# facebookresearch/flashy

Hardware: AMD Instinct MI355X
Metric: img/sec (higher is better)
Workload: dtype bf16; 1 GPU; model=resnet18, dataset=cifar10-shaped, global_batch=64, img_size=32, num_classes=10, parallelism=dp1, mode=native-kernels, graph=True, channels_last=False

## Files before the change

### flashy_amd/nn.py

```python
from __future__ import annotations

import math
import os
import typing as tp

import torch
from torch import nn

from . import ops


def _weight_bf16(w: torch.Tensor) -> torch.Tensor:
    mirror = getattr(w, "_bf16_mirror", None)
    if mirror is not None:
        return mirror
    return w.detach().to(torch.bfloat16)


def _grad_target(p: torch.Tensor) -> tp.Tuple[torch.Tensor, bool]:
    if p.grad is not None and p.grad.is_contiguous():
        return p.grad, True
    return torch.zeros_like(p, memory_format=torch.contiguous_format), False


# ... 63 lines not shown
                             self._wt_view, self.feeds_bn and self.training)


class WtCache:

    def __init__(self, model: nn.Module):
        convs = [m for m in model.modules()
                 if isinstance(m, Conv2d) and m.input_grad
                 and m.weight.shape[-1] % 64 == 0]
        metas, total = [], 0
        mirrors = [getattr(c.weight, "_bf16_mirror", None) for c in convs]
        if not convs or any(m is None for m in mirrors):
            self.meta = None
            return
        base = mirrors[0]
        for c, mir in zip(convs, mirrors):
            assert mir.untyped_storage().data_ptr() == \
                base.untyped_storage().data_ptr(), \
                "all conv weights must share one flat bf16 mirror"
            src_off = (mir.data_ptr() - base.data_ptr()) // 2
            assert src_off >= 0
            K, R, S, C = c.weight.shape
            metas.append((src_off, total, K, R * S * C))
            total += K * R * S * C
        dev = convs[0].weight.device
        self.src = mirrors[0]
        self.arena = torch.empty(total, dtype=torch.bfloat16, device=dev)
        self.meta = torch.tensor([list(m) for m in metas],
                                 dtype=torch.int32, device=dev).flatten()
        self.max_elems = max(m[2] * m[3] for m in metas)
        self.n = len(convs)
        for c, m in zip(convs, metas):
            K, R, S, C = c.weight.shape
            c._wt_view = self.arena[m[1]:m[1] + K * R * S * C].view(R, S, C, K)

    @property
    def active(self) -> bool:
        return self.meta is not None

    def refresh(self) -> None:
        if self.meta is not None:
            ops.weight_transpose_batched(self.src, self.arena, self.meta,
                                         self.n, self.max_elems)


class _BnFn(torch.autograd.Function):
    @staticmethod
    def forward(ctx, x: torch.Tensor, gamma: torch.Tensor, beta: torch.Tensor,
                res: tp.Optional[torch.Tensor], relu: bool, slope: float,
                module):
        N, H, W, C = x.shape
        M = N * H * W
        y = torch.empty_like(x)
        if module.training:
            fused = getattr(x, "_bn_stats", None)
            if fused is not None:
                partials, msplit = fused
            else:
                msplit = ops.bn_msplit(M, C)
                partials = torch.empty(msplit * 2 * C, dtype=torch.float32,
                                       device=x.device)
                ops.bn_stats(x, partials, M, C, msplit)
            work = torch.empty(4 * C, dtype=torch.float32, device=x.device)
            ops.bn_finalize(partials, msplit, gamma, beta, module.running_mean,
                            module.running_var, work, M, C, module.eps,
                            module.momentum, update_running=True)
        else:
            invstd = torch.rsqrt(module.running_var + module.eps)
            scale = gamma.detach() * invstd
            shift = beta.detach() - module.running_mean * scale
            work = torch.cat([module.running_mean, invstd, scale, shift])
        ops.bn_apply(x, res, y, work, M, C, relu, slope)
        ctx.save_for_backward(x, y, work)
        ctx.relu = relu
        ctx.slope = slope
        ctx.has_res = res is not None
        ctx.refs = (gamma, beta)
        return y

    @staticmethod
    def backward(ctx, dy: torch.Tensor):
        x, y, work = ctx.saved_tensors
        gamma, beta = ctx.refs
        N, H, W, C = x.shape
        M = N * H * W
        dy = dy.contiguous()
        msplit = ops.bn_msplit(M, C)
        partials = torch.empty(msplit * 2 * C, dtype=torch.float32,
                               device=x.device)
        bsums = torch.empty(2 * C, dtype=torch.float32, device=x.device)
        dz = torch.empty_like(dy)
        ops.bn_bwd_reduce(dy, y, x, work, dz, partials, M, C, msplit,
                          ctx.relu, ctx.slope)
        need_g, need_b = ctx.needs_input_grad[1], ctx.needs_input_grad[2]
        dgamma, g_direct = _grad_target(gamma) if need_g \
            else (torch.empty_like(gamma), True)
        dbeta, b_direct = _grad_target(beta) if need_b \
            else (torch.empty_like(beta), True)
        ops.bn_bwd_grads(partials, msplit, bsums, dgamma, dbeta, C)
        dx = torch.empty_like(x)
        ops.bn_bwd_apply(dz, x, work, bsums, dx, M, C)
        return (dx,
                dgamma if need_g and not g_direct else None,
                dbeta if need_b and not b_direct else None,
                dz if ctx.has_res else None,
                None, None, None)


class _ConvTransposeFn(torch.autograd.Function):

    @staticmethod
    def forward(ctx, x: torch.Tensor, w: torch.Tensor, stride: int, pad: int,
                input_grad: bool):
        w16 = _weight_bf16(w)
        N, Hi, Wi, Cin = x.shape
        K, R, S, Cout = w16.shape
        assert K == Cin, (x.shape, w16.shape)
        Ho = (Hi - 1) * stride - 2 * pad + R
        Wo = (Wi - 1) * stride - 2 * pad + S
        d = ops.ConvDims(N, Ho, Wo, Cout, Cin, R, S, Hi, Wi, stride, pad)
        y = x.new_empty((N, Ho, Wo, Cout))
        if Cout % 64 == 0:
            wt = w16.new_empty((R, S, Cout, Cin))
            ops.weight_transpose(w16, wt)
            ops.conv_dgrad(x, wt, y, d)
        else:
            ops.conv_stem_dgrad(x, w16, y, d)
        ctx.save_for_backward(x, w16)
        ctx.dims = d
        ctx.input_grad = input_grad
        ctx.w_ref = w
        return y

    @staticmethod
    def backward(ctx, dy: torch.Tensor):
        x, w16 = ctx.saved_tensors
        d: ops.ConvDims = ctx.dims
        dy = dy.contiguous()
        dw_buf = None
        direct = True
        if ctx.needs_input_grad[1]:
            dw_buf, direct = _grad_target(ctx.w_ref)
            ops.conv_wgrad(dy, x, dw_buf, d)
        dx = None
        if ctx.input_grad:
            dx = x.new_empty(x.shape)
            ops.conv_fwd(dy, w16, dx, d)
        return (dx, dw_buf if dw_buf is not None and not direct else None,
                None, None, None)


class ConvTranspose2d(nn.Module):

    def __init__(self, in_channels: int, out_channels: int, kernel_size: int,
# ... 220 lines not shown
```

### flashy_amd/ops/__init__.py

```python
from __future__ import annotations

import importlib.util
import math
import os
import typing as tp
from pathlib import Path

import torch

_ext = None
_load_error: tp.Optional[str] = None


def _find_so() -> tp.Optional[Path]:
    for pattern in ("_hip_ops*.so",):
        hits = sorted(Path(__file__).parent.glob(pattern))
        if hits:
            return hits[0]
    return None


def load_extension():
    global _ext, _load_error
    if _ext is not None:
# ... 631 lines not shown
        ext.conv_stem_wgrad(x.data_ptr(), dout.data_ptr(), dw.data_ptr(), *d,
                            _stream())



def bn_msplit(M: int, C: int) -> int:
    cols = max(1, C // 64)
    msplit = max(1, min(512 // cols, 512))
    msplit = max(1, min(msplit, (M + 31) // 32))
    if msplit >= 4:
        msplit &= ~3
    return msplit


def bn_stats(x: torch.Tensor, partials: torch.Tensor, M: int, C: int,
             msplit: int) -> None:
    require().bn_stats(x.data_ptr(), partials.data_ptr(), M, C, msplit, _stream())


def bn_finalize(partials, msplit: int, gamma, beta, rmean, rvar, work,
                M: int, C: int, eps: float, momentum: float,
                update_running: bool) -> None:
    require().bn_finalize(partials.data_ptr(), msplit, gamma.data_ptr(),
                          beta.data_ptr(), rmean.data_ptr(), rvar.data_ptr(),
                          work.data_ptr(), M, C, eps, momentum,
                          update_running, _stream())


def bn_apply(x, res, y, work, M: int, C: int, relu: bool,
             slope: float = 0.0) -> None:
    require().bn_apply(x.data_ptr(), res.data_ptr() if res is not None else 0,
                       y.data_ptr(), work.data_ptr(), M, C, relu, slope,
                       _stream())


def bn_bwd_reduce(dy, y, x, work, dz_out, partials, M: int, C: int,
                  msplit: int, relu: bool, slope: float = 0.0) -> None:
    require().bn_bwd_reduce(dy.data_ptr(), y.data_ptr(), x.data_ptr(),
                            work.data_ptr(), dz_out.data_ptr(),
                            partials.data_ptr(), M, C, msplit, relu, slope,
                            _stream())


def bn_bwd_grads(partials, msplit: int, bsums, dgamma, dbeta, C: int) -> None:
    require().bn_bwd_grads(partials.data_ptr(), msplit, bsums.data_ptr(),
                           dgamma.data_ptr(), dbeta.data_ptr(), C, _stream())


def bn_bwd_apply(dz, x, work, bsums, dx, M: int, C: int) -> None:
    require().bn_bwd_apply(dz.data_ptr(), x.data_ptr(), work.data_ptr(),
                           bsums.data_ptr(), dx.data_ptr(), M, C, _stream())



def cross_entropy_fwd_bwd(logits: torch.Tensor, target: torch.Tensor,
                          dlogits: torch.Tensor, loss_sum: torch.Tensor,
                          loss_scale: float, grad_scale: float) -> None:
    ext = require()
    B, C = logits.shape
    assert logits.is_contiguous() and target.dtype == torch.int64
    ext.cross_entropy(logits.data_ptr(), target.data_ptr(), dlogits.data_ptr(),
                      loss_sum.data_ptr(), B, C, loss_scale, grad_scale,
                      _is_bf16(logits), _stream())


def cross_entropy_mix_fwd_bwd(logits: torch.Tensor, target: torch.Tensor,
                              target_b: tp.Optional[torch.Tensor],
                              lam: tp.Optional[torch.Tensor],
                              dlogits: torch.Tensor, loss_sum: torch.Tensor,
                              label_smoothing: float, loss_scale: float,
                              grad_scale: float) -> None:
    ext = require()
    B, C = logits.shape
    assert logits.is_contiguous() and logits.is_cuda
    assert dlogits.is_contiguous() and dlogits.dtype == logits.dtype
    assert tuple(dlogits.shape) == (B, C)
    for t in (target, target_b):
        if t is not None:
            assert t.dtype == torch.int64 and tuple(t.shape) == (B,)
            assert t.is_contiguous() and t.device == logits.device
    if lam is not None:
        assert lam.dtype == torch.float32 and lam.numel() == 1
        assert lam.device == logits.device
    assert 0.0 <= label_smoothing <= 1.0, label_smoothing
    ext.cross_entropy_mix(logits.data_ptr(), target.data_ptr(),
                          target_b.data_ptr() if target_b is not None else 0,
                          lam.data_ptr() if lam is not None else 0,
                          dlogits.data_ptr(), loss_sum.data_ptr(), B, C,
                          float(label_smoothing), loss_scale, grad_scale,
                          _is_bf16(logits), _stream())


def bce_logits_fwd_bwd(x: torch.Tensor, dx: torch.Tensor,
                       loss_sum: torch.Tensor, target: float,
                       loss_scale: float, grad_scale: float) -> None:
    ext = require()
    assert x.is_contiguous()
    ext.bce_logits(x.data_ptr(), dx.data_ptr(), loss_sum.data_ptr(), x.numel(),
                   target, loss_scale, grad_scale, _is_bf16(x), _stream())


def mse_fwd_bwd(x: torch.Tensor, t: torch.Tensor, dx: torch.Tensor,
                loss_sum: torch.Tensor, loss_scale: float,
                grad_scale: float) -> None:
    ext = require()
    assert x.is_contiguous() and t.is_contiguous() and x.dtype == t.dtype
# ... 88 lines not shown
```

### flashy_amd/ops/csrc/batchnorm.hip

```cpp

#include "common.h"


__global__ void __launch_bounds__(256)
k_bn_stats(const uint16_t* __restrict__ x, float* __restrict__ partials,
           int64_t M, int C, int msplit, int m_per_block) {
    const int c8 = (threadIdx.x & 7) * 8;
    const int mlane = threadIdx.x >> 3;
    const int cbase = blockIdx.x * 64;
    const int64_t m0 = (int64_t)blockIdx.y * m_per_block;
    const int64_t m1 = min(m0 + (int64_t)m_per_block, M);
    float s[8] = {}, s2[8] = {};
    for (int64_t m = m0 + mlane; m < m1; m += 32) {
        const short8 v8 = *reinterpret_cast<const short8*>(
            x + m * C + cbase + c8);
#pragma unroll
        for (int j = 0; j < 8; ++j) {
            const float v = bf16_to_f32(((const uint16_t*)&v8)[j]);
            s[j] += v;
            s2[j] = fmaf(v, v, s2[j]);
        }
    }
    __shared__ float red[2][32][64];
#pragma unroll
// ... 2 lines not shown
        red[1][mlane][c8 + j] = s2[j];
    }
    __syncthreads();
    const int c = threadIdx.x & 63;
    const int which = threadIdx.x >> 6;
    if (which < 2) {
        float acc = 0.f;
#pragma unroll 8
        for (int i = 0; i < 32; ++i) acc += red[which][i][c];
        partials[((int64_t)which * C + cbase + c) * msplit + blockIdx.y] = acc;
    }
}


__device__ __forceinline__ void combine_partials8(
        const float* __restrict__ partials, int msplit, int C,
        float* s_out, float* s2_out) {
    const int ch = threadIdx.x & 7;
    const int slane = threadIdx.x >> 3;
    const int c = blockIdx.x * 8 + ch;
    const float* row0 = partials + (int64_t)c * msplit;
    const float* row1 = partials + ((int64_t)C + c) * msplit;
    float s = 0.f, s2 = 0.f;
    if (msplit & 3) {
        for (int i = slane; i < msplit; i += 32) {
            s += row0[i];
            s2 += row1[i];
        }
    } else {
        for (int i = slane * 4; i + 4 <= msplit; i += 128) {
            const float4 a = *reinterpret_cast<const float4*>(row0 + i);
            const float4 b = *reinterpret_cast<const float4*>(row1 + i);
            s += a.x + a.y + a.z + a.w;
            s2 += b.x + b.y + b.z + b.w;
        }
    }
    __shared__ float red[2][32][8];
    red[0][slane][ch] = s;
    red[1][slane][ch] = s2;
    __syncthreads();
    if (threadIdx.x < 16) {
        const int w = threadIdx.x >> 3;
        const int cc = threadIdx.x & 7;
        float acc = 0.f;
#pragma unroll 8
        for (int i = 0; i < 32; ++i) acc += red[w][i][cc];
        red[w][0][cc] = acc;
    }
    __syncthreads();
    *s_out = red[0][0][ch];
    *s2_out = red[1][0][ch];
}

__global__ void __launch_bounds__(256)
k_bn_finalize(const float* __restrict__ partials, int msplit,
              const float* __restrict__ gamma,
              const float* __restrict__ beta,
              float* __restrict__ running_mean,
              float* __restrict__ running_var,
              float* __restrict__ work, int64_t M, int C,
              float eps, float momentum, int update_running) {
    float s, s2;
    combine_partials8(partials, msplit, C, &s, &s2);
    if (threadIdx.x >= 8) return;
    const int c = blockIdx.x * 8 + threadIdx.x;
    const float mean = s / (float)M;
    float var = s2 / (float)M - mean * mean;
    var = fmaxf(var, 0.f);
    const float invstd = rsqrtf(var + eps);
    const float scale = gamma[c] * invstd;
    work[c] = mean;
    work[C + c] = invstd;
    work[2 * C + c] = scale;
    work[3 * C + c] = beta[c] - mean * scale;
    if (update_running) {
        running_mean[c] += momentum * (mean - running_mean[c]);
        const float unbiased = M > 1 ? var * (float)M / (float)(M - 1) : var;
        running_var[c] += momentum * (unbiased - running_var[c]);
    }
}


template <bool RELU, bool RES>
__global__ void __launch_bounds__(256)
k_bn_apply(const uint16_t* __restrict__ x, const uint16_t* __restrict__ res,
           uint16_t* __restrict__ y, const float* __restrict__ work,
           int64_t M, int C, float slope) {
    const int64_t total8 = M * C / 8;
    const int64_t stride = (int64_t)gridDim.x * blockDim.x;
    const float4* scale4 = reinterpret_cast<const float4*>(work + 2 * (int64_t)C);
    const float4* shift4 = reinterpret_cast<const float4*>(work + 3 * (int64_t)C);
    for (int64_t i = (int64_t)blockIdx.x * blockDim.x + threadIdx.x; i < total8;
         i += stride) {
        const int co = (int)((i * 8) % C) / 4;
        const float4 sc[2] = {scale4[co], scale4[co + 1]};
        const float4 sh[2] = {shift4[co], shift4[co + 1]};
        short8 xv = *reinterpret_cast<const short8*>(x + i * 8);
        short8 rv = {};
        if (RES) rv = *reinterpret_cast<const short8*>(res + i * 8);
        short8 out;
#pragma unroll
        for (int j = 0; j < 8; ++j) {
            float v = fmaf(bf16_to_f32(((const uint16_t*)&xv)[j]),
                           ((const float*)sc)[j], ((const float*)sh)[j]);
            if (RES) v += bf16_to_f32(((const uint16_t*)&rv)[j]);
            if (RELU) v = v > 0.f ? v : slope * v;
            ((uint16_t*)&out)[j] = f32_to_bf16(v);
        }
        *reinterpret_cast<short8*>(y + i * 8) = out;
    }
}

template <bool RELU, bool RES>
__global__ void __launch_bounds__(256)
k_bn_apply_c64(const uint16_t* __restrict__ x, const uint16_t* __restrict__ res,
               uint16_t* __restrict__ y, const float* __restrict__ work,
               int64_t M, int C, float slope, int m_per_block) {
    const int c = blockIdx.x * 64 + (threadIdx.x & 7) * 8;
    const int mlane = threadIdx.x >> 3;
    const int64_t m0 = (int64_t)blockIdx.y * m_per_block;
    const int64_t m1 = min(m0 + (int64_t)m_per_block, M);
    float sc[8], sh[8];
#pragma unroll
    for (int j = 0; j < 8; ++j) {
        sc[j] = work[2 * (int64_t)C + c + j];
        sh[j] = work[3 * (int64_t)C + c + j];
    }
    for (int64_t m = m0 + mlane; m < m1; m += 32) {
        const int64_t off = m * C + c;
        short8 xv = *reinterpret_cast<const short8*>(x + off);
        short8 rv = {};
        if (RES) rv = *reinterpret_cast<const short8*>(res + off);
        short8 out;
#pragma unroll
        for (int j = 0; j < 8; ++j) {
            float v = fmaf(bf16_to_f32(((const uint16_t*)&xv)[j]), sc[j], sh[j]);
            if (RES) v += bf16_to_f32(((const uint16_t*)&rv)[j]);
            if (RELU) v = v > 0.f ? v : slope * v;
            ((uint16_t*)&out)[j] = f32_to_bf16(v);
        }
        *reinterpret_cast<short8*>(y + off) = out;
    }
}

__global__ void __launch_bounds__(256)
k_bn_bwd_apply_c64(const uint16_t* __restrict__ dz,
                   const uint16_t* __restrict__ x,
                   const float* __restrict__ work,
                   const float* __restrict__ bsums,
                   uint16_t* __restrict__ dx, int64_t M, int C,
                   int m_per_block) {
    const int c = blockIdx.x * 64 + (threadIdx.x & 7) * 8;
    const int mlane = threadIdx.x >> 3;
    const int64_t m0 = (int64_t)blockIdx.y * m_per_block;
    const int64_t m1 = min(m0 + (int64_t)m_per_block, M);
    const float invM = 1.f / (float)M;
    float mn[8], is[8], sc[8], b0[8], b1[8];
#pragma unroll
    for (int j = 0; j < 8; ++j) {
        mn[j] = work[c + j];
        is[j] = work[C + c + j];
        sc[j] = work[2 * (int64_t)C + c + j];
        b0[j] = bsums[c + j] * invM;
        b1[j] = bsums[C + c + j] * invM;
    }
    for (int64_t m = m0 + mlane; m < m1; m += 32) {
        const int64_t off = m * C + c;
        short8 gz = *reinterpret_cast<const short8*>(dz + off);
        short8 xv = *reinterpret_cast<const short8*>(x + off);
        short8 out;
#pragma unroll
        for (int j = 0; j < 8; ++j) {
            const float xhat = (bf16_to_f32(((const uint16_t*)&xv)[j]) - mn[j])
                               * is[j];
            const float g = bf16_to_f32(((const uint16_t*)&gz)[j]);
            ((uint16_t*)&out)[j] =
                f32_to_bf16(sc[j] * (g - b0[j] - xhat * b1[j]));
        }
        *reinterpret_cast<short8*>(dx + off) = out;
    }
}

static inline int apply_mpb(int64_t M, int C) {
    const int cblocks = C / 64;
    int target = 1024 / cblocks;
    if (target < 1) target = 1;
    int64_t mblocks = (M + 31) / 32;
    if (mblocks > target) mblocks = target;
    return (int)((M + mblocks - 1) / mblocks);
}


template <bool RELU>
__global__ void __launch_bounds__(256)
k_bn_bwd_reduce(const uint16_t* __restrict__ dy, const uint16_t* __restrict__ y,
                const uint16_t* __restrict__ x, const float* __restrict__ work,
                uint16_t* __restrict__ dz_out, float* __restrict__ partials,
                int64_t M, int C, int msplit, int m_per_block, float slope) {
    const int c8 = (threadIdx.x & 7) * 8;
    const int mlane = threadIdx.x >> 3;
    const int cbase = blockIdx.x * 64;
    const int64_t m0 = (int64_t)blockIdx.y * m_per_block;
    const int64_t m1 = min(m0 + (int64_t)m_per_block, M);
    float mean[8], invstd[8];
#pragma unroll
    for (int j = 0; j < 8; ++j) {
        mean[j] = work[cbase + c8 + j];
        invstd[j] = work[C + cbase + c8 + j];
    }
    float s[8] = {}, sx[8] = {};
    for (int64_t m = m0 + mlane; m < m1; m += 32) {
        const int64_t off = m * C + cbase + c8;
        const short8 g8 = *reinterpret_cast<const short8*>(dy + off);
        const short8 x8 = *reinterpret_cast<const short8*>(x + off);
        short8 y8 = {};
        if (RELU) y8 = *reinterpret_cast<const short8*>(y + off);
        short8 dz8;
#pragma unroll
        for (int j = 0; j < 8; ++j) {
            float g = bf16_to_f32(((const uint16_t*)&g8)[j]);
            if (RELU && bf16_to_f32(((const uint16_t*)&y8)[j]) <= 0.f)
                g *= slope;
            ((uint16_t*)&dz8)[j] = f32_to_bf16(g);
            s[j] += g;
            const float xh = (bf16_to_f32(((const uint16_t*)&x8)[j]) - mean[j]) * invstd[j];
            sx[j] = fmaf(g, xh, sx[j]);
        }
        *reinterpret_cast<short8*>(dz_out + off) = dz8;
    }
    __shared__ float red[2][32][64];
#pragma unroll
// ... 11 lines not shown
        partials[((int64_t)which * C + cbase + c) * msplit + blockIdx.y] = acc;
    }
}

__global__ void __launch_bounds__(256)
k_bn_bwd_grads(const float* __restrict__ partials, int msplit,
               float* __restrict__ bsums,
               float* __restrict__ dgamma,
               float* __restrict__ dbeta, int C) {
    float s, sx;
    combine_partials8(partials, msplit, C, &s, &sx);
    if (threadIdx.x >= 8) return;
    const int c = blockIdx.x * 8 + threadIdx.x;
    bsums[c] = s;
    bsums[C + c] = sx;
    dbeta[c] += s;
    dgamma[c] += sx;
}


__global__ void __launch_bounds__(256)
k_bn_bwd_apply(const uint16_t* __restrict__ dz, const uint16_t* __restrict__ x,
               const float* __restrict__ work, const float* __restrict__ bsums,
               uint16_t* __restrict__ dx, int64_t M, int C) {
    const int64_t total8 = M * C / 8;
    const int64_t stride = (int64_t)gridDim.x * blockDim.x;
    const float invM = 1.f / (float)M;
    const float4* mean4 = reinterpret_cast<const float4*>(work);
    const float4* invstd4 = reinterpret_cast<const float4*>(work + C);
    const float4* scale4 = reinterpret_cast<const float4*>(work + 2 * (int64_t)C);
    const float4* b04 = reinterpret_cast<const float4*>(bsums);
    const float4* b14 = reinterpret_cast<const float4*>(bsums + C);
    for (int64_t i = (int64_t)blockIdx.x * blockDim.x + threadIdx.x; i < total8;
         i += stride) {
        const int co = (int)((i * 8) % C) / 4;
        const float4 mn[2] = {mean4[co], mean4[co + 1]};
        const float4 is[2] = {invstd4[co], invstd4[co + 1]};
        const float4 sc[2] = {scale4[co], scale4[co + 1]};
        const float4 b0[2] = {b04[co], b04[co + 1]};
        const float4 b1[2] = {b14[co], b14[co + 1]};
        short8 gz = *reinterpret_cast<const short8*>(dz + i * 8);
        short8 xv = *reinterpret_cast<const short8*>(x + i * 8);
        short8 out;
#pragma unroll
        for (int j = 0; j < 8; ++j) {
            const float xhat = (bf16_to_f32(((const uint16_t*)&xv)[j]) -
                                ((const float*)mn)[j]) * ((const float*)is)[j];
            const float g = bf16_to_f32(((const uint16_t*)&gz)[j]);
            const float v = ((const float*)sc)[j] *
                (g - (((const float*)b0)[j] + xhat * ((const float*)b1)[j]) * invM);
            ((uint16_t*)&out)[j] = f32_to_bf16(v);
        }
        *reinterpret_cast<short8*>(dx + i * 8) = out;
    }
}


extern "C" void launch_bn_stats(const void* x, void* partials, int64_t M, int C,
                                int msplit, hipStream_t stream) {
    const int mpb = (int)((M + msplit - 1) / msplit);
    dim3 grid((unsigned)(C / 64), (unsigned)msplit);
    k_bn_stats<<<grid, 256, 0, stream>>>((const uint16_t*)x, (float*)partials,
                                         M, C, msplit, mpb);
}

extern "C" void launch_bn_finalize(const void* partials, int msplit,
                                   const void* gamma, const void* beta,
                                   void* running_mean, void* running_var,
                                   void* work, int64_t M, int C, float eps,
                                   float momentum, int update_running,
                                   hipStream_t stream) {
    k_bn_finalize<<<C / 8, 256, 0, stream>>>(
        (const float*)partials, msplit, (const float*)gamma,
        (const float*)beta, (float*)running_mean, (float*)running_var,
        (float*)work, M, C, eps, momentum, update_running);
}

extern "C" void launch_bn_apply(const void* x, const void* res, void* y,
                                const void* work, int64_t M, int C, int relu,
                                float slope, hipStream_t stream) {
    if (C % 64 == 0) {
        const int mpb = apply_mpb(M, C);
        dim3 g((unsigned)(C / 64), (unsigned)((M + mpb - 1) / mpb));
        if (relu && res)
            k_bn_apply_c64<true, true><<<g, 256, 0, stream>>>(
                (const uint16_t*)x, (const uint16_t*)res, (uint16_t*)y,
                (const float*)work, M, C, slope, mpb);
        else if (relu)
            k_bn_apply_c64<true, false><<<g, 256, 0, stream>>>(
                (const uint16_t*)x, nullptr, (uint16_t*)y,
                (const float*)work, M, C, slope, mpb);
        else if (res)
            k_bn_apply_c64<false, true><<<g, 256, 0, stream>>>(
                (const uint16_t*)x, (const uint16_t*)res, (uint16_t*)y,
                (const float*)work, M, C, slope, mpb);
        else
            k_bn_apply_c64<false, false><<<g, 256, 0, stream>>>(
                (const uint16_t*)x, nullptr, (uint16_t*)y,
                (const float*)work, M, C, slope, mpb);
        return;
    }
    const int grid = ew_grid(M * C / 8, 256, 4);
    if (relu && res)
        k_bn_apply<true, true><<<grid, 256, 0, stream>>>(
            (const uint16_t*)x, (const uint16_t*)res, (uint16_t*)y,
            (const float*)work, M, C, slope);
// ... 3 lines not shown
    else if (res)
        k_bn_apply<false, true><<<grid, 256, 0, stream>>>(
            (const uint16_t*)x, (const uint16_t*)res, (uint16_t*)y,
            (const float*)work, M, C, slope);
    else
        k_bn_apply<false, false><<<grid, 256, 0, stream>>>(
            (const uint16_t*)x, nullptr, (uint16_t*)y, (const float*)work, M, C, slope);
}

extern "C" void launch_bn_bwd_reduce(const void* dy, const void* y,
                                     const void* x, const void* work,
                                     void* dz_out, void* partials, int64_t M,
                                     int C, int msplit, int relu, float slope,
                                     hipStream_t stream) {
    const int mpb = (int)((M + msplit - 1) / msplit);
    dim3 grid((unsigned)(C / 64), (unsigned)msplit);
    if (relu)
        k_bn_bwd_reduce<true><<<grid, 256, 0, stream>>>(
            (const uint16_t*)dy, (const uint16_t*)y, (const uint16_t*)x,
            (const float*)work, (uint16_t*)dz_out, (float*)partials, M, C,
            msplit, mpb, slope);
    else
        k_bn_bwd_reduce<false><<<grid, 256, 0, stream>>>(
            (const uint16_t*)dy, (const uint16_t*)y, (const uint16_t*)x,
            (const float*)work, (uint16_t*)dz_out, (float*)partials, M, C,
            msplit, mpb, slope);
}

extern "C" void launch_bn_bwd_grads(const void* partials, int msplit,
                                    void* bsums, void* dgamma, void* dbeta,
                                    int C, hipStream_t stream) {
    k_bn_bwd_grads<<<C / 8, 256, 0, stream>>>(
        (const float*)partials, msplit, (float*)bsums, (float*)dgamma,
        (float*)dbeta, C);
}

extern "C" void launch_bn_bwd_apply(const void* dz, const void* x,
                                    const void* work, const void* bsums,
                                    void* dx, int64_t M, int C,
                                    hipStream_t stream) {
    if (C % 64 == 0) {
        const int mpb = apply_mpb(M, C);
        dim3 g((unsigned)(C / 64), (unsigned)((M + mpb - 1) / mpb));
        k_bn_bwd_apply_c64<<<g, 256, 0, stream>>>(
            (const uint16_t*)dz, (const uint16_t*)x, (const float*)work,
            (const float*)bsums, (uint16_t*)dx, M, C, mpb);
        return;
    }
    const int grid = ew_grid(M * C / 8, 256, 4);
    k_bn_bwd_apply<<<grid, 256, 0, stream>>>(
        (const uint16_t*)dz, (const uint16_t*)x, (const float*)work,
        (const float*)bsums, (uint16_t*)dx, M, C);
}
```

### flashy_amd/ops/csrc/ext.cpp

```cpp

#include <hip/hip_runtime.h>
#include <pybind11/pybind11.h>
#include <pybind11/stl.h>

#include <cstdint>
#include <stdexcept>
#include <vector>

#include "conv8.h"

namespace py = pybind11;

extern "C" {
void launch_conv_fwd(const void* x, const void* w, void* y, ConvDims d,
                     int relu, void* bn_ws, hipStream_t stream);
int conv_fwd_msplit(ConvDims d);
void launch_stem_pad_x(const void* x, void* xp, int64_t N, int H, int W,
                       int Hp, int Wp, int pad, hipStream_t stream);
void launch_stem_pad_w(const void* w, void* wp, int K, int R, int S,
                       hipStream_t stream);
void launch_stem_unpad_dw(const void* dwp, void* dw, int K, int R, int S,
                          hipStream_t stream);
void launch_conv_stem_fwd(const void* x, const void* w, void* y, ConvDims d,
                          hipStream_t stream);
void launch_conv_stem_wgrad(const void* x, const void* dout, void* dw,
                            ConvDims d, hipStream_t stream);
void launch_conv_stem_dgrad(const void* dout, const void* w, void* dx,
                            ConvDims d, hipStream_t stream);
void launch_conv_dgrad(const void* dout, const void* w_rsck, void* dx,
                       ConvDims d, hipStream_t stream);
void launch_conv_fwd_splitk(const void* x, const void* w, void* ws, ConvDims d,
                            int zn, hipStream_t stream);
void launch_conv_dgrad_splitk(const void* dout, const void* w_rsck, void* ws,
                              ConvDims d, int zn, hipStream_t stream);
void launch_splitk_combine(const void* ws, void* out, int64_t total, int zn,
                           int relu, hipStream_t stream);
void launch_splitk_combine_stats(const void* ws, void* out, void* partials,
                                 int64_t M, int K, int zn, int msplit,
                                 hipStream_t stream);
void launch_pool_fc_fwd(const void* x, const void* w, const void* b,
                        void* pooled, void* y, int N, int HW, int C, int O,
                        hipStream_t stream);
void launch_head_dw(const void* pooled, const void* dy, void* dw, void* db,
                    int B, int C, int O, hipStream_t stream);
void launch_head_dx(const void* dy, const void* w, void* dx, int N, int HW,
                    int C, int O, hipStream_t stream);
void launch_weight_transpose(const void* w, void* wt, int K, int rsc,
                             hipStream_t stream);
void launch_weight_transpose_batched(const void* src, void* dst,
                                     const void* meta, int n_convs,
                                     int64_t max_elems, hipStream_t stream);
void launch_conv_wgrad(const void* x, const void* dout, void* dw, ConvDims d,
                       int n_splits, hipStream_t stream);
void launch_bn_stats(const void* x, void* partials, int64_t M, int C,
                     int msplit, hipStream_t stream);
void launch_bn_finalize(const void* partials, int msplit, const void* gamma,
                        const void* beta, void* running_mean,
                        void* running_var, void* work, int64_t M, int C,
                        float eps, float momentum, int update_running,
                        hipStream_t stream);
void launch_bn_apply(const void* x, const void* res, void* y, const void* work,
                     int64_t M, int C, int relu, float slope,
                     hipStream_t stream);
void launch_bn_bwd_reduce(const void* dy, const void* y, const void* x,
                          const void* work, void* dz_out, void* partials,
                          int64_t M, int C, int msplit, int relu, float slope,
                          hipStream_t stream);
void launch_bn_bwd_grads(const void* partials, int msplit, void* bsums,
                         void* dgamma, void* dbeta, int C, hipStream_t stream);
void launch_bn_bwd_apply(const void* dz, const void* x, const void* work,
                         const void* bsums, void* dx, int64_t M, int C,
                         hipStream_t stream);
void launch_fused_sgd(void* p, const void* g, void* m, void* p_bf16, int64_t n,
                      float lr, float momentum, float wd, float grad_scale,
                      int nesterov, const void* hyper, hipStream_t stream);
void launch_fused_adam(void* p, const void* g, void* m, void* v, void* p_bf16,
                       void* step_dev, int64_t n, float lr, float beta1,
                       float beta2, float eps, float wd, int64_t step,
                       float grad_scale, int adamw, const void* hyper,
                       hipStream_t stream);
void launch_adam_step_inc(void* p, hipStream_t stream);
int grad_sqsum_blocks(int64_t n);
void launch_grad_sqsum(const void* g, int64_t n, void* partials,
                       hipStream_t stream);
void launch_optim_prepare(void* hyper, const void* partials, int n_partials,
                          const void* step_dev, double max_norm, int kind,
                          double base_lr, int64_t warmup_steps,
                          double start_factor, int64_t total_steps,
                          double min_ratio, const int64_t* milestones,
                          int n_milestones, double gamma, hipStream_t stream);
void launch_seg_sqsum(const void* p, const void* g, const void* chunks,
                      int n_chunks, void* partials, hipStream_t stream);
void launch_lars_prepare(const void* partials, const void* tensor_chunk,
                         const void* wd, const void* lars_on, void* ratio,
                         int n_tensors, const void* hyper, float grad_scale,
                         double eta, double eps, hipStream_t stream);
void launch_fused_sgd_seg(void* p, const void* g, void* m, void* p_bf16,
                          int64_t n, float lr, float momentum,
                          float grad_scale, int nesterov, const void* hyper,
                          const void* chunks, int n_chunks, const void* wd,
                          const void* lr_scale, const void* ratio,
                          hipStream_t stream);
void launch_fused_adam_seg(void* p, const void* g, void* m, void* v,
                           void* p_bf16, void* step_dev, int64_t n, float lr,
                           float beta1, float beta2, float eps, int64_t step,
                           float grad_scale, int adamw, const void* hyper,
                           const void* chunks, int n_chunks, const void* wd,
                           const void* lr_scale, hipStream_t stream);
void launch_image_ingest(const void* src, void* out, const void* step_dev,
                         int N, int H, int W, int OH, int OW, int pad,
                         uint64_t seed, uint32_t flip_thresh,
                         const float* scale, const float* bias, int fill,
                         int train, hipStream_t stream);
void launch_resized_crop_draw(void* boxes, const void* tables,
                              const void* step_dev, int N, int H, int W,
                              int OH, int OW, uint64_t seed, uint64_t root_hw,
                              uint32_t flip_thresh, uint32_t r0, uint32_t r1,
                              uint32_t eval_crop, int train,
                              hipStream_t stream);
void launch_resized_crop(const void* src, void* out, const void* boxes, int N,
                         int H, int W, int OH, int OW, const float* scale,
                         const float* bias, hipStream_t stream);
void launch_batch_mix_draw(void* row, const void* lam_table,
                           const void* sq_table, const void* step_dev, int H,
                           int W, uint64_t seed, uint32_t prob_thresh,
// ... 229 lines not shown
    m.def("bn_stats",
          [](uintptr_t x, uintptr_t partials, int64_t M, int C, int msplit,
             uintptr_t stream) {
              launch_bn_stats((const void*)x, (void*)partials, M, C, msplit,
                              as_stream(stream));
              check_last();
          });
    m.def("bn_finalize",
          [](uintptr_t partials, int msplit, uintptr_t gamma, uintptr_t beta,
             uintptr_t rmean, uintptr_t rvar, uintptr_t work, int64_t M, int C,
             float eps, float momentum, bool update_running, uintptr_t stream) {
              launch_bn_finalize((const void*)partials, msplit,
                                 (const void*)gamma, (const void*)beta,
                                 (void*)rmean, (void*)rvar, (void*)work, M, C,
                                 eps, momentum, update_running ? 1 : 0,
                                 as_stream(stream));
              check_last();
          });
    m.def("bn_apply",
          [](uintptr_t x, uintptr_t res, uintptr_t y, uintptr_t work, int64_t M,
             int C, bool relu, float slope, uintptr_t stream) {
              launch_bn_apply((const void*)x, (const void*)res, (void*)y,
                              (const void*)work, M, C, relu ? 1 : 0, slope,
                              as_stream(stream));
              check_last();
          });
    m.def("bn_bwd_reduce",
          [](uintptr_t dy, uintptr_t y, uintptr_t x, uintptr_t work,
             uintptr_t dz_out, uintptr_t partials, int64_t M, int C,
             int msplit, bool relu, float slope, uintptr_t stream) {
              launch_bn_bwd_reduce((const void*)dy, (const void*)y,
                                   (const void*)x, (const void*)work,
                                   (void*)dz_out, (void*)partials, M, C,
                                   msplit, relu ? 1 : 0, slope,
                                   as_stream(stream));
              check_last();
          });
    m.def("bn_bwd_grads",
          [](uintptr_t partials, int msplit, uintptr_t bsums, uintptr_t dgamma,
             uintptr_t dbeta, int C, uintptr_t stream) {
              launch_bn_bwd_grads((const void*)partials, msplit, (void*)bsums,
                                  (void*)dgamma, (void*)dbeta, C,
                                  as_stream(stream));
              check_last();
          });
    m.def("bn_bwd_apply",
          [](uintptr_t dz, uintptr_t x, uintptr_t work, uintptr_t bsums,
             uintptr_t dx, int64_t M, int C, uintptr_t stream) {
              launch_bn_bwd_apply((const void*)dz, (const void*)x,
                                  (const void*)work, (const void*)bsums,
                                  (void*)dx, M, C, as_stream(stream));
              check_last();
          });

    m.def("fused_sgd",
          [](uintptr_t p, uintptr_t g, uintptr_t mom, uintptr_t p_bf16,
             int64_t n, float lr, float momentum, float wd, float grad_scale,
             bool nesterov, uintptr_t stream, uintptr_t hyper) {
              launch_fused_sgd((void*)p, (const void*)g, (void*)mom,
                               (void*)p_bf16, n, lr, momentum, wd, grad_scale,
                               nesterov ? 1 : 0, (const void*)hyper,
                               as_stream(stream));
              check_last();
          },
          py::arg("p"), py::arg("g"), py::arg("mom"), py::arg("p_bf16"),
          py::arg("n"), py::arg("lr"), py::arg("momentum"), py::arg("wd"),
          py::arg("grad_scale"), py::arg("nesterov"), py::arg("stream"),
          py::arg("hyper") = (uintptr_t)0);

    m.def("fused_adam",
          [](uintptr_t p, uintptr_t g, uintptr_t mom, uintptr_t var,
             uintptr_t p_bf16, uintptr_t step_dev, int64_t n, float lr,
             float beta1, float beta2, float eps, float wd, int64_t step,
             float grad_scale, bool adamw, uintptr_t stream,
             uintptr_t hyper) {
              launch_fused_adam((void*)p, (const void*)g, (void*)mom,
                                (void*)var, (void*)p_bf16, (void*)step_dev, n,
                                lr, beta1, beta2, eps, wd, step, grad_scale,
                                adamw ? 1 : 0, (const void*)hyper,
                                as_stream(stream));
              check_last();
          },
          py::arg("p"), py::arg("g"), py::arg("mom"), py::arg("var"),
          py::arg("p_bf16"), py::arg("step_dev"), py::arg("n"), py::arg("lr"),
          py::arg("beta1"), py::arg("beta2"), py::arg("eps"), py::arg("wd"),
          py::arg("step"), py::arg("grad_scale"), py::arg("adamw"),
          py::arg("stream"), py::arg("hyper") = (uintptr_t)0);
    m.def("adam_step_inc", [](uintptr_t p, uintptr_t stream) {
        launch_adam_step_inc((void*)p, as_stream(stream));
        check_last();
    });
    m.def("grad_sqsum_blocks", [](int64_t n) { return grad_sqsum_blocks(n); });
    m.def("grad_sqsum",
          [](uintptr_t g, int64_t n, uintptr_t partials, uintptr_t stream) {
              launch_grad_sqsum((const void*)g, n, (void*)partials,
                                as_stream(stream));
              check_last();
          });
    m.def("optim_prepare",
          [](uintptr_t hyper, uintptr_t partials, int n_partials,
             uintptr_t step_dev, double max_norm, int kind, double base_lr,
             int64_t warmup_steps, double start_factor, int64_t total_steps,
             double min_ratio, const std::vector<int64_t>& milestones,
             double gamma, uintptr_t stream) {
              if (milestones.size() > 8)
                  throw std::invalid_argument("at most 8 milestones");
// ... 268 lines not shown
```

Baseline: 31270 img/s.

## Fuse small-shape batchnorm finalize+apply and backward chain into single kernels

For batchnorm layers with few rows (M up to 512 forward, up to 1024 backward), the forward finalize and apply steps now run in one kernel. The backward reduce, grads and apply steps also collapse into one per-channel-group kernel that keeps rows in registers and reduces through shared memory. This cuts kernel launches and repeated global reads of dy, x and y on the small late-stage ResNet layers. The trade-off is low parallelism: one block per 8 channels, and the backward kernel adds into dgamma/dbeta directly.

```diff
diff --git a/flashy_amd/nn.py b/flashy_amd/nn.py
--- a/flashy_amd/nn.py
+++ b/flashy_amd/nn.py
@@ -139,6 +139,8 @@
         N, H, W, C = x.shape
         M = N * H * W
         y = torch.empty_like(x)
+        fwd_form, bwd_form = ops.bn_small_plan(M, C) if module.training \
+            else ("chain", "chain")
         if module.training:
             fused = getattr(x, "_bn_stats", None)
             if fused is not None:
@@ -149,18 +151,27 @@
                                        device=x.device)
                 ops.bn_stats(x, partials, M, C, msplit)
             work = torch.empty(4 * C, dtype=torch.float32, device=x.device)
-            ops.bn_finalize(partials, msplit, gamma, beta, module.running_mean,
-                            module.running_var, work, M, C, module.eps,
-                            module.momentum, update_running=True)
+            if fwd_form == "small":
+                ops.bn_fwd_small(partials, msplit, gamma, beta,
+                                 module.running_mean, module.running_var, work,
+                                 x, res, y, M, C, module.eps, module.momentum,
+                                 True, relu, slope)
+            else:
+                ops.bn_finalize(partials, msplit, gamma, beta,
+                                module.running_mean, module.running_var, work,
+                                M, C, module.eps, module.momentum,
+                                update_running=True)
         else:
             invstd = torch.rsqrt(module.running_var + module.eps)
             scale = gamma.detach() * invstd
             shift = beta.detach() - module.running_mean * scale
             work = torch.cat([module.running_mean, invstd, scale, shift])
-        ops.bn_apply(x, res, y, work, M, C, relu, slope)
+        if fwd_form != "small":
+            ops.bn_apply(x, res, y, work, M, C, relu, slope)
         ctx.save_for_backward(x, y, work)
         ctx.relu = relu
         ctx.slope = slope
+        ctx.bwd_form = bwd_form
         ctx.has_res = res is not None
         ctx.refs = (gamma, beta)
         return y
@@ -172,21 +183,27 @@
         N, H, W, C = x.shape
         M = N * H * W
         dy = dy.contiguous()
-        msplit = ops.bn_msplit(M, C)
-        partials = torch.empty(msplit * 2 * C, dtype=torch.float32,
-                               device=x.device)
-        bsums = torch.empty(2 * C, dtype=torch.float32, device=x.device)
-        dz = torch.empty_like(dy)
-        ops.bn_bwd_reduce(dy, y, x, work, dz, partials, M, C, msplit,
-                          ctx.relu, ctx.slope)
         need_g, need_b = ctx.needs_input_grad[1], ctx.needs_input_grad[2]
         dgamma, g_direct = _grad_target(gamma) if need_g \
             else (torch.empty_like(gamma), True)
         dbeta, b_direct = _grad_target(beta) if need_b \
             else (torch.empty_like(beta), True)
-        ops.bn_bwd_grads(partials, msplit, bsums, dgamma, dbeta, C)
         dx = torch.empty_like(x)
-        ops.bn_bwd_apply(dz, x, work, bsums, dx, M, C)
+        if ctx.bwd_form != "chain":
+            dz = torch.empty_like(dy) if ctx.has_res else None
+            ops.bn_bwd_small(dy, y, x, work, dz, dgamma, dbeta, dx, M, C,
+                             ctx.relu, ctx.slope, write_dz=ctx.has_res,
+                             form=ctx.bwd_form)
+        else:
+            msplit = ops.bn_msplit(M, C)
+            partials = torch.empty(msplit * 2 * C, dtype=torch.float32,
+                                   device=x.device)
+            bsums = torch.empty(2 * C, dtype=torch.float32, device=x.device)
+            dz = torch.empty_like(dy)
+            ops.bn_bwd_reduce(dy, y, x, work, dz, partials, M, C, msplit,
+                              ctx.relu, ctx.slope)
+            ops.bn_bwd_grads(partials, msplit, bsums, dgamma, dbeta, C)
+            ops.bn_bwd_apply(dz, x, work, bsums, dx, M, C)
         return (dx,
                 dgamma if need_g and not g_direct else None,
                 dbeta if need_b and not b_direct else None,
diff --git a/flashy_amd/ops/__init__.py b/flashy_amd/ops/__init__.py
--- a/flashy_amd/ops/__init__.py
+++ b/flashy_amd/ops/__init__.py
@@ -707,6 +707,42 @@
                            bsums.data_ptr(), dx.data_ptr(), M, C, _stream())
 
 
+BN_BWD_SMALL_FORMS = {"chain": 0, "regs8": 1}
+
+
+def bn_small_plan(M: int, C: int) -> tp.Tuple[str, str]:
+    fwd, bwd = require().bn_small_plan(M, C)
+    names = {v: k for k, v in BN_BWD_SMALL_FORMS.items()}
+    return ("small" if fwd else "chain"), names[bwd]
+
+
+def bn_fwd_small(partials, msplit: int, gamma, beta, rmean, rvar, work, x,
+                 res, y, M: int, C: int, eps: float, momentum: float,
+                 update_running: bool, relu: bool, slope: float = 0.0) -> None:
+    assert x.is_contiguous() and y.is_contiguous() and x.numel() == M * C
+    assert res is None or res.is_contiguous()
+    require().bn_fwd_small(
+        partials.data_ptr(), msplit, gamma.data_ptr(), beta.data_ptr(),
+        rmean.data_ptr(), rvar.data_ptr(), work.data_ptr(), x.data_ptr(),
+        res.data_ptr() if res is not None else 0, y.data_ptr(), M, C, eps,
+        momentum, update_running, relu, slope, 1, _stream())
+
+
+def bn_bwd_small(dy, y, x, work, dz, dgamma, dbeta, dx, M: int, C: int,
+                 relu: bool, slope: float = 0.0, write_dz: bool = True,
+                 form: str = "regs8") -> None:
+    assert all(t.is_contiguous() for t in (dy, y, x, dx))
+    assert x.numel() == M * C
+    assert dz.is_contiguous() if write_dz else True
+    if form == "chain":
+        raise ValueError("bn_bwd_small: 'chain' is not a single-kernel form")
+    require().bn_bwd_small(
+        dy.data_ptr(), y.data_ptr(), x.data_ptr(), work.data_ptr(),
+        dz.data_ptr() if dz is not None else 0, dgamma.data_ptr(),
+        dbeta.data_ptr(), dx.data_ptr(),
+        M, C, relu, slope, write_dz, BN_BWD_SMALL_FORMS[form], _stream())
+
+
 
 def cross_entropy_fwd_bwd(logits: torch.Tensor, target: torch.Tensor,
                           dlogits: torch.Tensor, loss_sum: torch.Tensor,
diff --git a/flashy_amd/ops/csrc/batchnorm.hip b/flashy_amd/ops/csrc/batchnorm.hip
--- a/flashy_amd/ops/csrc/batchnorm.hip
+++ b/flashy_amd/ops/csrc/batchnorm.hip
@@ -78,6 +78,32 @@
     *s2_out = red[1][0][ch];
 }
 
+__device__ __forceinline__ void bn_finalize_channel(
+        float s, float s2, int c,
+        const float* __restrict__ gamma, const float* __restrict__ beta,
+        float* __restrict__ running_mean, float* __restrict__ running_var,
+        float* __restrict__ work, int64_t M, int C,
+        float eps, float momentum, int update_running,
+        float* scale_out, float* shift_out) {
+    const float mean = s / (float)M;
+    float var = s2 / (float)M - mean * mean;
+    var = fmaxf(var, 0.f);
+    const float invstd = rsqrtf(var + eps);
+    const float scale = gamma[c] * invstd;
+    const float shift = beta[c] - mean * scale;
+    work[c] = mean;
+    work[C + c] = invstd;
+    work[2 * C + c] = scale;
+    work[3 * C + c] = shift;
+    if (update_running) {
+        running_mean[c] += momentum * (mean - running_mean[c]);
+        const float unbiased = M > 1 ? var * (float)M / (float)(M - 1) : var;
+        running_var[c] += momentum * (unbiased - running_var[c]);
+    }
+    *scale_out = scale;
+    *shift_out = shift;
+}
+
 __global__ void __launch_bounds__(256)
 k_bn_finalize(const float* __restrict__ partials, int msplit,
               const float* __restrict__ gamma,
@@ -89,21 +115,10 @@
     float s, s2;
     combine_partials8(partials, msplit, C, &s, &s2);
     if (threadIdx.x >= 8) return;
-    const int c = blockIdx.x * 8 + threadIdx.x;
-    const float mean = s / (float)M;
-    float var = s2 / (float)M - mean * mean;
-    var = fmaxf(var, 0.f);
-    const float invstd = rsqrtf(var + eps);
-    const float scale = gamma[c] * invstd;
-    work[c] = mean;
-    work[C + c] = invstd;
-    work[2 * C + c] = scale;
-    work[3 * C + c] = beta[c] - mean * scale;
-    if (update_running) {
-        running_mean[c] += momentum * (mean - running_mean[c]);
-        const float unbiased = M > 1 ? var * (float)M / (float)(M - 1) : var;
-        running_var[c] += momentum * (unbiased - running_var[c]);
-    }
+    float scale, shift;
+    bn_finalize_channel(s, s2, blockIdx.x * 8 + threadIdx.x, gamma, beta,
+                        running_mean, running_var, work, M, C, eps, momentum,
+                        update_running, &scale, &shift);
 }
 
 
@@ -138,6 +153,24 @@
 }
 
 template <bool RELU, bool RES>
+__device__ __forceinline__ uint16_t bn_apply_elem(uint16_t x, uint16_t r,
+                                                  float sc, float sh,
+                                                  float slope) {
+    float v = fmaf(bf16_to_f32(x), sc, sh);
+    if (RES) v += bf16_to_f32(r);
+    if (RELU) v = v > 0.f ? v : slope * v;
+    return f32_to_bf16(v);
+}
+
+__device__ __forceinline__ uint16_t bn_bwd_dx_elem(uint16_t dz, uint16_t x,
+                                                   float mn, float is, float sc,
+                                                   float b0, float b1) {
+    const float xhat = (bf16_to_f32(x) - mn) * is;
+    const float g = bf16_to_f32(dz);
+    return f32_to_bf16(sc * (g - b0 - xhat * b1));
+}
+
+template <bool RELU, bool RES>
 __global__ void __launch_bounds__(256)
 k_bn_apply_c64(const uint16_t* __restrict__ x, const uint16_t* __restrict__ res,
                uint16_t* __restrict__ y, const float* __restrict__ work,
@@ -159,12 +192,10 @@
         if (RES) rv = *reinterpret_cast<const short8*>(res + off);
         short8 out;
 #pragma unroll
-        for (int j = 0; j < 8; ++j) {
-            float v = fmaf(bf16_to_f32(((const uint16_t*)&xv)[j]), sc[j], sh[j]);
-            if (RES) v += bf16_to_f32(((const uint16_t*)&rv)[j]);
-            if (RELU) v = v > 0.f ? v : slope * v;
-            ((uint16_t*)&out)[j] = f32_to_bf16(v);
-        }
+        for (int j = 0; j < 8; ++j)
+            ((uint16_t*)&out)[j] = bn_apply_elem<RELU, RES>(
+                ((const uint16_t*)&xv)[j], ((const uint16_t*)&rv)[j],
+                sc[j], sh[j], slope);
         *reinterpret_cast<short8*>(y + off) = out;
     }
 }
@@ -196,13 +227,10 @@
         short8 xv = *reinterpret_cast<const short8*>(x + off);
         short8 out;
 #pragma unroll
-        for (int j = 0; j < 8; ++j) {
-            const float xhat = (bf16_to_f32(((const uint16_t*)&xv)[j]) - mn[j])
-                               * is[j];
-            const float g = bf16_to_f32(((const uint16_t*)&gz)[j]);
-            ((uint16_t*)&out)[j] =
-                f32_to_bf16(sc[j] * (g - b0[j] - xhat * b1[j]));
-        }
+        for (int j = 0; j < 8; ++j)
+            ((uint16_t*)&out)[j] = bn_bwd_dx_elem(
+                ((const uint16_t*)&gz)[j], ((const uint16_t*)&xv)[j],
+                mn[j], is[j], sc[j], b0[j], b1[j]);
         *reinterpret_cast<short8*>(dx + off) = out;
     }
 }
@@ -320,6 +348,185 @@
             ((uint16_t*)&out)[j] = f32_to_bf16(v);
         }
         *reinterpret_cast<short8*>(dx + i * 8) = out;
+    }
+}
+
+
+template <bool RELU, bool RES>
+__global__ void __launch_bounds__(256)
+k_bn_fwd_small(const float* __restrict__ partials, int msplit,
+               const float* __restrict__ gamma, const float* __restrict__ beta,
+               float* __restrict__ running_mean,
+               float* __restrict__ running_var, float* __restrict__ work,
+               const uint16_t* __restrict__ x, const uint16_t* __restrict__ res,
+               uint16_t* __restrict__ y, int64_t M, int C, float eps,
+               float momentum, int update_running, float slope) {
+    const int c0 = blockIdx.x * 8;
+    short8 xv[4] = {}, rv[4] = {};
+#pragma unroll
+    for (int r = 0; r < 4; ++r) {
+        const int64_t m = threadIdx.x + 256 * r;
+        if (m < M) {
+            xv[r] = *reinterpret_cast<const short8*>(x + m * C + c0);
+            if (RES) rv[r] = *reinterpret_cast<const short8*>(res + m * C + c0);
+        }
+    }
+    float s, s2;
+    combine_partials8(partials, msplit, C, &s, &s2);
+    __shared__ float coef[2][8];
+    if (threadIdx.x < 8) {
+        float scale, shift;
+        bn_finalize_channel(s, s2, c0 + threadIdx.x, gamma, beta, running_mean,
+                            running_var, work, M, C, eps, momentum,
+                            update_running, &scale, &shift);
+        coef[0][threadIdx.x] = scale;
+        coef[1][threadIdx.x] = shift;
+    }
+    __syncthreads();
+    float sc[8], sh[8];
+#pragma unroll
+    for (int j = 0; j < 8; ++j) {
+        sc[j] = coef[0][j];
+        sh[j] = coef[1][j];
+    }
+#pragma unroll
+    for (int r = 0; r < 4; ++r) {
+        const int64_t m = threadIdx.x + 256 * r;
+        if (m < M) {
+            short8 out;
+#pragma unroll
+            for (int j = 0; j < 8; ++j)
+                ((uint16_t*)&out)[j] = bn_apply_elem<RELU, RES>(
+                    ((const uint16_t*)&xv[r])[j], ((const uint16_t*)&rv[r])[j],
+                    sc[j], sh[j], slope);
+            *reinterpret_cast<short8*>(y + m * C + c0) = out;
+        }
+    }
+    for (int64_t m = threadIdx.x + 1024; m < M; m += 256) {
+        const int64_t off = m * C + c0;
+        const short8 xr = *reinterpret_cast<const short8*>(x + off);
+        short8 rr = {};
+        if (RES) rr = *reinterpret_cast<const short8*>(res + off);
+        short8 out;
+#pragma unroll
+        for (int j = 0; j < 8; ++j)
+            ((uint16_t*)&out)[j] = bn_apply_elem<RELU, RES>(
+                ((const uint16_t*)&xr)[j], ((const uint16_t*)&rr)[j],
+                sc[j], sh[j], slope);
+        *reinterpret_cast<short8*>(y + off) = out;
+    }
+}
+
+template <int CW> struct bn_vec {
+    using type = __attribute__((ext_vector_type(CW))) short;
+};
+
+template <bool RELU, int CW>
+__device__ __forceinline__ void bn_bwd_row(
+        const uint16_t* __restrict__ dy, const uint16_t* __restrict__ y,
+        const uint16_t* __restrict__ x, int64_t off, const float* mean,
+        const float* invstd, float slope, float* s, float* sx,
+        typename bn_vec<CW>::type* dz_out, typename bn_vec<CW>::type* x_out) {
+    using vec = typename bn_vec<CW>::type;
+    const vec gv = *reinterpret_cast<const vec*>(dy + off);
+    const vec xv = *reinterpret_cast<const vec*>(x + off);
+    vec yv = {};
+    if (RELU) yv = *reinterpret_cast<const vec*>(y + off);
+    vec dzv;
+#pragma unroll
+    for (int j = 0; j < CW; ++j) {
+        float g = bf16_to_f32(((const uint16_t*)&gv)[j]);
+        if (RELU && bf16_to_f32(((const uint16_t*)&yv)[j]) <= 0.f)
+            g *= slope;
+        ((uint16_t*)&dzv)[j] = f32_to_bf16(g);
+        s[j] += g;
+        const float xh = (bf16_to_f32(((const uint16_t*)&xv)[j]) - mean[j]) * invstd[j];
+        sx[j] = fmaf(g, xh, sx[j]);
+    }
+    *dz_out = dzv;
+    *x_out = xv;
+}
+
+template <bool RELU, bool WRITE_DZ, int CW, int R>
+__global__ void __launch_bounds__(256)
+k_bn_bwd_small(const uint16_t* __restrict__ dy, const uint16_t* __restrict__ y,
+               const uint16_t* __restrict__ x, const float* __restrict__ work,
+               uint16_t* __restrict__ dz_out, float* __restrict__ dgamma,
+               float* __restrict__ dbeta, uint16_t* __restrict__ dx,
+               int64_t M, int C, float slope) {
+    using vec = typename bn_vec<CW>::type;
+    constexpr int NQ = 128 / CW;
+    int grp = blockIdx.x;
+    if (gridDim.x % 8 == 0)
+        grp = (blockIdx.x & 7) * (gridDim.x >> 3) + (blockIdx.x >> 3);
+    const int c0 = grp * CW;
+    const int t = threadIdx.x;
+    float mean[CW], invstd[CW];
+#pragma unroll
+    for (int j = 0; j < CW; ++j) {
+        mean[j] = work[c0 + j];
+        invstd[j] = work[C + c0 + j];
+    }
+    float s[CW] = {}, sx[CW] = {};
+    vec dzk[R], xk[R];
+#pragma unroll
+    for (int r = 0; r < R; ++r) {
+        const int64_t m = t + 256 * r;
+        if (m < M) {
+            const int64_t off = m * C + c0;
+            bn_bwd_row<RELU, CW>(dy, y, x, off, mean, invstd, slope, s, sx,
+                                 &dzk[r], &xk[r]);
+            if (WRITE_DZ) *reinterpret_cast<vec*>(dz_out + off) = dzk[r];
+        }
+    }
+    __shared__ float red[2][256][CW];
+    __shared__ float red2[2][NQ][CW];
+    __shared__ float fin[2][CW];
+#pragma unroll
+    for (int j = 0; j < CW; ++j) {
+        red[0][t][j] = s[j];
+        red[1][t][j] = sx[j];
+    }
+    __syncthreads();
+    {
+        const int kind = t >> 7, q = t & 127;
+        const int k = q / CW, ch = q % CW;
+        float acc = 0.f;
+#pragma unroll
+        for (int i = 0; i < 256 / NQ; ++i) acc += red[kind][k + NQ * i][ch];
+        red2[kind][k][ch] = acc;
+    }
+    __syncthreads();
+    if (t < 2 * CW) {
+        const int kind = t / CW, ch = t % CW;
+        float acc = 0.f;
+#pragma unroll 8
+        for (int k = 0; k < NQ; ++k) acc += red2[kind][k][ch];
+        fin[kind][ch] = acc;
+        if (kind == 0) dbeta[c0 + ch] += acc;
+        else dgamma[c0 + ch] += acc;
+    }
+    __syncthreads();
+    const float invM = 1.f / (float)M;
+    float sc[CW], b0[CW], b1[CW];
+#pragma unroll
+    for (int j = 0; j < CW; ++j) {
+        sc[j] = work[2 * (int64_t)C + c0 + j];
+        b0[j] = fin[0][j] * invM;
+        b1[j] = fin[1][j] * invM;
+    }
+#pragma unroll
+    for (int r = 0; r < R; ++r) {
+        const int64_t m = t + 256 * r;
+        if (m < M) {
+            vec out;
+#pragma unroll
+            for (int j = 0; j < CW; ++j)
+                ((uint16_t*)&out)[j] = bn_bwd_dx_elem(
+                    ((const uint16_t*)&dzk[r])[j], ((const uint16_t*)&xk[r])[j],
+                    mean[j], invstd[j], sc[j], b0[j], b1[j]);
+            *reinterpret_cast<vec*>(dx + m * C + c0) = out;
+        }
     }
 }
 
@@ -429,3 +636,75 @@
         (const uint16_t*)dz, (const uint16_t*)x, (const float*)work,
         (const float*)bsums, (uint16_t*)dx, M, C);
 }
+
+
+static inline int bn_bwd_small_rows(int64_t M) {
+    return M <= 1024 ? 4 : M <= 4096 ? 16 : 0;
+}
+
+extern "C" void bn_small_plan(int64_t M, int C, int* fwd_form, int* bwd_form) {
+    *fwd_form = 0;
+    *bwd_form = 0;
+    if (M < 1 || C < 8 || C % 8) return;
+    if (M <= 512) *fwd_form = 1;
+    if (M <= 1024) *bwd_form = 1;
+}
+
+extern "C" int launch_bn_fwd_small(const void* partials, int msplit,
+                                   const void* gamma, const void* beta,
+                                   void* running_mean, void* running_var,
+                                   void* work, const void* x, const void* res,
+                                   void* y, int64_t M, int C, float eps,
+                                   float momentum, int update_running,
+                                   int relu, float slope, int form,
+                                   hipStream_t stream) {
+    if (form != 1 || M < 1 || C < 8 || C % 8) return 0;
+#define BN_FWD_SMALL(RELU, RES)                                               \
+    k_bn_fwd_small<RELU, RES><<<C / 8, 256, 0, stream>>>(                     \
+        (const float*)partials, msplit, (const float*)gamma,                  \
+        (const float*)beta, (float*)running_mean, (float*)running_var,        \
+        (float*)work, (const uint16_t*)x, (const uint16_t*)res, (uint16_t*)y, \
+        M, C, eps, momentum, update_running, slope)
+    if (relu && res) BN_FWD_SMALL(true, true);
+    else if (relu) BN_FWD_SMALL(true, false);
+    else if (res) BN_FWD_SMALL(false, true);
+    else BN_FWD_SMALL(false, false);
+#undef BN_FWD_SMALL
+    return 1;
+}
+
+template <int CW, int R>
+static void bn_bwd_small_launch(const void* dy, const void* y, const void* x,
+                                const void* work, void* dz, void* dgamma,
+                                void* dbeta, void* dx, int64_t M, int C,
+                                int relu, float slope, int write_dz,
+                                hipStream_t stream) {
+#define BN_BWD_SMALL(RELU, WDZ)                                               \
+    k_bn_bwd_small<RELU, WDZ, CW, R><<<C / CW, 256, 0, stream>>>(             \
+        (const uint16_t*)dy, (const uint16_t*)y, (const uint16_t*)x,          \
+        (const float*)work, (uint16_t*)dz, (float*)dgamma, (float*)dbeta,     \
+        (uint16_t*)dx, M, C, slope)
+    if (relu && write_dz) BN_BWD_SMALL(true, true);
+    else if (relu) BN_BWD_SMALL(true, false);
+    else if (write_dz) BN_BWD_SMALL(false, true);
+    else BN_BWD_SMALL(false, false);
+#undef BN_BWD_SMALL
+}
+
+extern "C" int launch_bn_bwd_small(const void* dy, const void* y,
+                                   const void* x, const void* work, void* dz,
+                                   void* dgamma, void* dbeta, void* dx,
+                                   int64_t M, int C, int relu, float slope,
+                                   int write_dz, int form,
+                                   hipStream_t stream) {
+    if (form != 1 || M < 1 || C < 8 || C % 8) return 0;
+    const int rows = bn_bwd_small_rows(M);
+    if (!rows) return 0;
+#define BN_BWD_GO(CW, R)                                                      \
+    bn_bwd_small_launch<CW, R>(dy, y, x, work, dz, dgamma, dbeta, dx, M, C,   \
+                               relu, slope, write_dz, stream)
+    if (rows == 4) BN_BWD_GO(8, 4);
+    else BN_BWD_GO(8, 16);
+#undef BN_BWD_GO
+    return 1;
+}
diff --git a/flashy_amd/ops/csrc/ext.cpp b/flashy_amd/ops/csrc/ext.cpp
--- a/flashy_amd/ops/csrc/ext.cpp
+++ b/flashy_amd/ops/csrc/ext.cpp
@@ -71,6 +71,17 @@
 void launch_bn_bwd_apply(const void* dz, const void* x, const void* work,
                          const void* bsums, void* dx, int64_t M, int C,
                          hipStream_t stream);
+void bn_small_plan(int64_t M, int C, int* fwd_form, int* bwd_form);
+int launch_bn_fwd_small(const void* partials, int msplit, const void* gamma,
+                        const void* beta, void* running_mean,
+                        void* running_var, void* work, const void* x,
+                        const void* res, void* y, int64_t M, int C, float eps,
+                        float momentum, int update_running, int relu,
+                        float slope, int form, hipStream_t stream);
+int launch_bn_bwd_small(const void* dy, const void* y, const void* x,
+                        const void* work, void* dz, void* dgamma, void* dbeta,
+                        void* dx, int64_t M, int C, int relu, float slope,
+                        int write_dz, int form, hipStream_t stream);
 void launch_fused_sgd(void* p, const void* g, void* m, void* p_bf16, int64_t n,
                       float lr, float momentum, float wd, float grad_scale,
                       int nesterov, const void* hyper, hipStream_t stream);
@@ -406,6 +417,41 @@
                                   (void*)dx, M, C, as_stream(stream));
               check_last();
           });
+    m.def("bn_small_plan", [](int64_t M, int C) {
+        int fwd = 0, bwd = 0;
+        bn_small_plan(M, C, &fwd, &bwd);
+        return py::make_tuple(fwd, bwd);
+    });
+    m.def("bn_fwd_small",
+          [](uintptr_t partials, int msplit, uintptr_t gamma, uintptr_t beta,
+             uintptr_t rmean, uintptr_t rvar, uintptr_t work, uintptr_t x,
+             uintptr_t res, uintptr_t y, int64_t M, int C, float eps,
+             float momentum, bool update_running, bool relu, float slope,
+             int form, uintptr_t stream) {
+              if (!launch_bn_fwd_small(
+                      (const void*)partials, msplit, (const void*)gamma,
+                      (const void*)beta, (void*)rmean, (void*)rvar,
+                      (void*)work, (const void*)x, (const void*)res, (void*)y,
+                      M, C, eps, momentum, update_running ? 1 : 0,
+                      relu ? 1 : 0, slope, form, as_stream(stream)))
+                  throw std::invalid_argument(
+                      "bn_fwd_small: form cannot run this shape");
+              check_last();
+          });
+    m.def("bn_bwd_small",
+          [](uintptr_t dy, uintptr_t y, uintptr_t x, uintptr_t work,
+             uintptr_t dz, uintptr_t dgamma, uintptr_t dbeta, uintptr_t dx,
+             int64_t M, int C, bool relu, float slope, bool write_dz, int form,
+             uintptr_t stream) {
+              if (!launch_bn_bwd_small(
+                      (const void*)dy, (const void*)y, (const void*)x,
+                      (const void*)work, (void*)dz, (void*)dgamma,
+                      (void*)dbeta, (void*)dx, M, C, relu ? 1 : 0, slope,
+                      write_dz ? 1 : 0, form, as_stream(stream)))
+                  throw std::invalid_argument(
+                      "bn_bwd_small: form cannot run this shape");
+              check_last();
+          });
 
     m.def("fused_sgd",
           [](uintptr_t p, uintptr_t g, uintptr_t mom, uintptr_t p_bf16,
```

Result: faster. 31600 img/s (median of 6 runs) (+1.0%).
